# Roywangj/AdaptPoint

Measured on AMD Instinct MI355X. Metric: set-abstraction fwd+bwd point-clouds/sec (B=32,N=1024), higher is better.
Workload: dtype bf16

## Files before the change

### adaptpoint_amd/csrc/sa_fused.hip

```cpp
#include "apn_common.h"
#include "apn_mfma.h"
#include <type_traits>
#include "sa_chain.h"

namespace apn {

constexpr int SA_C = 32;
constexpr int SA_C1 = 32;
constexpr int SA_C2 = 64;
constexpr int SA_K = 32;
constexpr int SA_WAVES = 4;

template <int NS>
__device__ __forceinline__ void put_frag(uint4 *base, int f, int lane, const Frag<NS> &v) {
#pragma unroll
    for (int p = 0; p < NS; ++p) base[(f * NS + p) * 64 + lane] = __builtin_bit_cast(uint4, v.p[p]);
}

template <int NS>
__device__ __forceinline__ Frag<NS> get_frag(const uint4 *base, int f, int lane) {
    Frag<NS> v;
#pragma unroll
    for (int p = 0; p < NS; ++p) v.p[p] = __builtin_bit_cast(bf16x8, base[(f * NS + p) * 64 + lane]);
    return v;
}

template <int NS>
__device__ __forceinline__ float eff(float v) {
    const __bf16 hi = (__bf16)v;
    float r = (float)hi;
    if (NS == 2) r += (float)(__bf16)(v - r);
    return r;
}

struct SaArgs {
    int b, n, m;
    const float *xyz;
    const float *new_xyz;
    const __bf16 *ft;
    const __bf16 *ft_lo;
    const int *idx;
    const float *w1;
    float radius;
    const int *tmap;
    unsigned long long *stamps;
};

__device__ __forceinline__ void stamp(const SaArgs &a, int wave, int k) {
    if (a.stamps && (threadIdx.x & 63) == 0)
        a.stamps[((size_t)blockIdx.x * SA_WAVES + wave) * 16 + k] = wall_clock64();
}

__device__ __forceinline__ int tm_tiles(const SaArgs &a) { return a.tmap[0]; }
__device__ __forceinline__ const int *tm_tq0(const SaArgs &a) { return a.tmap + 4; }
__device__ __forceinline__ const unsigned *tm_rows(const SaArgs &a) {
    return reinterpret_cast<const unsigned *>(a.tmap + 4 + ((a.b * a.m + 3) & ~3));
}
__device__ __forceinline__ const int *tm_nn(const SaArgs &a) {
    return a.tmap + 4 + ((a.b * a.m + 3) & ~3) + (size_t)32 * a.b * a.m;
}
__device__ __forceinline__ unsigned ri_q(unsigned info) { return info & 0xffu; }
__device__ __forceinline__ unsigned ri_slot(unsigned info) { return (info >> 8) & 0xffu; }
__device__ __forceinline__ unsigned ri_mult(unsigned info) { return (info >> 16) & 0xffu; }
__device__ __forceinline__ void row_meta(unsigned info, int h, unsigned (&meta)[16]) {
#pragma unroll
    for (int i = 0; i < 16; ++i) meta[i] = (unsigned)__builtin_amdgcn_ds_bpermute(acc_row(i, h) << 2, (int)info);
}

template <int NS>
__device__ __forceinline__ void load_w1_frags(const float *__restrict__ w1, int r, int h,
                                              Frag<NS> (&wf)[3]) {
#pragma unroll
    for (int s = 0; s < 3; ++s) {
        float t[8];
#pragma unroll
        for (int j = 0; j < 8; ++j)
            t[j] = s < 2 ? w1[r * 35 + 3 + 16 * s + 8 * h + j]
                         : ((h == 0 && j < 3) ? w1[r * 35 + j] : 0.0f);
        wf[s] = make_frag<NS>(t);
    }
}

constexpr int PS_PTS = 512, PS_MAX_ROWS = 64, PS_NT = 2 * PS_PTS;
constexpr double GEO_INV_UNIT = 1.0 / 68719476736.0;

#ifdef APN_WG_STAMPS
__device__ unsigned long long *d_wg_stamps_f = nullptr;
__device__ __forceinline__ void wg_stamp(int k) {
    unsigned long long *st = d_wg_stamps_f;
    if (st && threadIdx.x == 0) st[(size_t)blockIdx.x * 16 + k] = wall_clock64();
}
#else
__device__ __forceinline__ void wg_stamp(int) {}
#endif

template <int NS>
__global__ __launch_bounds__(PS_NT) void sa_prep_stats_kernel(
    int n, int tiles_per_cloud, int total_tiles, const float *__restrict__ f, const long long *__restrict__ geo,
    const double *__restrict__ dd, int dd_rows, const float *__restrict__ w1, int stats, __bf16 *__restrict__ ft,
    __bf16 *__restrict__ ft_lo, float *__restrict__ part, unsigned long long *__restrict__ zero, long long zero_words) {
    extern __shared__ float sf_raw[];
    float (*sf)[PS_PTS + 1] = reinterpret_cast<float (*)[PS_PTS + 1]>(sf_raw);
    __shared__ float4 sgeo[PS_PTS];
    __shared__ float red[PS_NT / 64][64];
    __shared__ double sdd[6];
    const int tid = threadIdx.x, lane = tid & 63, r = lane & 31, h = lane >> 5;
    const int wave = __builtin_amdgcn_readfirstlane(tid >> 6);
    critical_stream_priority();
    wg_stamp(0);
    for (long long e = (long long)blockIdx.x * PS_NT + tid; e < zero_words; e += (long long)gridDim.x * PS_NT) zero[e] = 0ull;
    Frag<NS> wf[3];
    load_w1_frags<NS>(w1, r, h, wf);
    const float wp0 = eff<NS>(w1[r * 35]), wp1 = eff<NS>(w1[r * 35 + 1]), wp2 = eff<NS>(w1[r * 35 + 2]);
    float s1 = 0.0f, s2 = 0.0f;
    for (int tile = blockIdx.x; tile < total_tiles; tile += gridDim.x) {
        const int cloud = tile / tiles_per_cloud, n0 = (tile % tiles_per_cloud) * PS_PTS;
        {
            const int pt = tid & (PS_PTS - 1), cg = tid / PS_PTS;
            const bool in = n0 + pt < n;
            float v[16];
#pragma unroll
            for (int k = 0; k < 16; ++k) v[k] = in ? f[((size_t)cloud * SA_C + cg + 2 * k) * n + n0 + pt] : 0.0f;
            float4 gv = make_float4(0.f, 0.f, 0.f, 0.f);
            if (stats && in && cg == 0) {
                const longlong2 *gp = reinterpret_cast<const longlong2 *>(geo + ((size_t)cloud * n + n0 + pt) * 4);
                const longlong2 g0 = gp[0], g1 = gp[1];
                gv = make_float4((float)g0.x, (float)((double)g0.y * GEO_INV_UNIT), (float)((double)g1.x * GEO_INV_UNIT),
                                 (float)((double)g1.y * GEO_INV_UNIT));
            }
            wg_stamp(1);
            __syncthreads();
#pragma unroll
            for (int k = 0; k < 16; ++k) sf[cg + 2 * k][pt] = v[k];
            if (cg == 0) sgeo[pt] = gv;
            wg_stamp(2);
        }
        __syncthreads();
        wg_stamp(3);
        const int pt = 32 * wave + r;
        float x0[8], x1[8];
#pragma unroll
        for (int j = 0; j < 8; ++j) { x0[j] = sf[8 * h + j][pt]; x1[j] = sf[16 + 8 * h + j][pt]; }
        const Frag<NS> a0 = make_frag<NS>(x0), a1 = make_frag<NS>(x1);
        if (n0 + pt < n) {
            uint4 *row = reinterpret_cast<uint4 *>(ft + ((size_t)cloud * n + n0 + pt) * SA_C);
            row[h] = __builtin_bit_cast(uint4, a0.p[0]);
            row[2 + h] = __builtin_bit_cast(uint4, a1.p[0]);
            if (NS == 2) {
                uint4 *rl = reinterpret_cast<uint4 *>(ft_lo + ((size_t)cloud * n + n0 + pt) * SA_C);
                rl[h] = __builtin_bit_cast(uint4, a0.p[NS - 1]);
                rl[2 + h] = __builtin_bit_cast(uint4, a1.p[NS - 1]);
            }
        }
        wg_stamp(4);
        if (stats) {
            f32x16 y = {0};
            y = mfma<NS>(a0, wf[0], y);
            y = mfma<NS>(a1, wf[1], y);
#pragma unroll
            for (int i = 0; i < 16; ++i) {
                const float4 g = sgeo[32 * wave + acc_row(i, h)];
                const float PD = __builtin_fmaf(wp2, g.w, __builtin_fmaf(wp1, g.z, wp0 * g.y));
                const float oF = g.x * y[i];
                s1 += oF + PD;
                s2 += __builtin_fmaf(oF, y[i], 2.0f * y[i] * PD);
            }
        }
    }
    wg_stamp(5);
    if (!stats) return;
    s1 += __shfl_xor(s1, 32);
    s2 += __shfl_xor(s2, 32);
    if (lane < 32) { red[wave][r] = s1; red[wave][32 + r] = s2; }
    if (blockIdx.x == 0 && wave >= 1 && wave < 7) {
        double s = 0.0;
        for (int e = lane; e < dd_rows; e += 64) s += dd[(size_t)e * 6 + (wave - 1)];
#pragma unroll
        for (int o = 32; o > 0; o >>= 1) s += __shfl_xor(s, o);
        if (lane == 0) sdd[wave - 1] = s;
    }
    __syncthreads();
    if (tid < 64) {
        float val = 0.0f;
#pragma unroll
        for (int w = 0; w < PS_NT / 64; ++w) val += red[w][tid];
        if (tid >= 32 && blockIdx.x == 0) {
            const double wx = wp0, wy = wp1, wz = wp2;
            const double t = wx * wx * sdd[0] + 2.0 * wx * wy * sdd[1] + 2.0 * wx * wz * sdd[2] + wy * wy * sdd[3] +
                             2.0 * wy * wz * sdd[4] + wz * wz * sdd[5];
            val += (float)t;
        }
        part[(size_t)blockIdx.x * 64 + tid] = val;
    }
    wg_stamp(6);
}

template <int NS>
struct TileRaw {
    uint4 f[2], fl[NS];
    float px, py, pz;
    float qx, qy, qz;
    int nb;
    unsigned info;
    int q0;
};

struct TileHead {
    int nb, q0;
    unsigned info;
    int tile;
};
template <bool CP>
__device__ __forceinline__ TileHead load_head(const SaArgs &a, int tile, int r) {
    TileHead t;
    t.tile = tile;
    if (CP) {
        t.nb = tm_nn(a)[(size_t)tile * SA_K + r];
        t.info = tm_rows(a)[(size_t)tile * SA_K + r];
        t.q0 = tm_tq0(a)[tile];
    } else {
        t.nb = a.idx[(size_t)tile * SA_K + r];
        t.info = 0x10000u | ((unsigned)r << 8);
        t.q0 = tile;
    }
    return t;
}

template <typename T>
__device__ __forceinline__ T ld_off(const void *base, unsigned byte_off) {
    return *reinterpret_cast<const T *>(reinterpret_cast<const char *>(base) + byte_off);
}

template <int NS>
__device__ __forceinline__ void fetch_tile(const SaArgs &a, const TileHead &hd, int h, TileRaw<NS> &t) {
    const int nb = hd.nb;
    const unsigned cloud = (unsigned)(hd.q0 / a.m);
    const unsigned pt = cloud * (unsigned)a.n + (unsigned)nb;
    const unsigned rowoff = pt * (unsigned)(SA_C * 2) + 16u * (unsigned)h;
    t.f[0] = ld_off<uint4>(a.ft, rowoff);
    t.f[1] = ld_off<uint4>(a.ft, rowoff + 32u);
    if (NS == 2) {
        t.fl[0] = ld_off<uint4>(a.ft_lo, rowoff);
        t.fl[NS - 1] = ld_off<uint4>(a.ft_lo, rowoff + 32u);
    }
    struct xyz3 { float x, y, z; };
    const xyz3 pp = ld_off<xyz3>(a.xyz, pt * 12u);
    t.px = pp.x; t.py = pp.y; t.pz = pp.z;
    const unsigned q = (unsigned)hd.q0 + (ri_mult(hd.info) ? ri_q(hd.info) : 0u);
    const xyz3 qq = ld_off<xyz3>(a.new_xyz, q * 12u);
    t.qx = qq.x; t.qy = qq.y; t.qz = qq.z;
    t.nb = nb;
    t.info = hd.info;
    t.q0 = hd.q0;
}

template <int NS>
__device__ __forceinline__ void build_frags(const SaArgs &a, const TileRaw<NS> &t, int h,
                                            Frag<NS> (&x)[3], float *deff = nullptr) {
    x[0].p[0] = __builtin_bit_cast(bf16x8, t.f[0]);
    x[1].p[0] = __builtin_bit_cast(bf16x8, t.f[1]);
    if (NS == 2) {
        x[0].p[NS - 1] = __builtin_bit_cast(bf16x8, t.fl[0]);
        x[1].p[NS - 1] = __builtin_bit_cast(bf16x8, t.fl[NS - 1]);
    }
    float d[8] = {0.f, 0.f, 0.f, 0.f, 0.f, 0.f, 0.f, 0.f};
    if (h == 0 || deff) {
        d[0] = (t.px - t.qx) / a.radius;
        d[1] = (t.py - t.qy) / a.radius;
        d[2] = (t.pz - t.qz) / a.radius;
    }
    if (deff) {
#pragma unroll
        for (int j = 0; j < 3; ++j) {
            const __bf16 hi = (__bf16)d[j];
            deff[j] = (float)hi;
            if (NS == 2) deff[j] += (float)(__bf16)(d[j] - (float)hi);
        }
        if (h != 0) d[0] = d[1] = d[2] = 0.0f;
    }
    x[2] = make_frag<NS>(d);
}

__device__ __forceinline__ void touch(const TileHead &hd) {
    asm volatile("" ::"v"(hd.nb), "v"(hd.info), "v"(hd.q0));
}

struct NoAhead {
    __device__ __forceinline__ void operator()(const TileHead &) const {}
};
template <int NS, bool CP, bool LATE = false, typename Pro, typename Pre, typename Body, typename Ahead = NoAhead>
__device__ __forceinline__ void for_each_tile(const SaArgs &a, int wave, int r, int h, Pro prologue, Pre pre, Body body,
                                              Ahead ahead = Ahead()) {
    const int cap = a.b * a.m, stride = gridDim.x * SA_WAVES;
    const int tiles = CP ? tm_tiles(a) : cap;
    const bool xcd = (gridDim.x & 7) == 0;
    const int per_x = (tiles + 7) >> 3;
    auto remap = [&](int t) {
        if (!xcd) return t;
        const int wg = t / SA_WAVES, wv = t - wg * SA_WAVES;
        const int x = wg & 7, u = (wg >> 3) * SA_WAVES + wv;
        return u < per_x ? x * per_x + u : tiles;
    };
    int slot = blockIdx.x * SA_WAVES + wave;
    int tile = remap(slot);
    const TileHead hd0 = load_head<CP>(a, tile < tiles ? tile : 0, r);
    TileHead hd_nxt = load_head<CP>(a, remap(slot + stride) < tiles ? remap(slot + stride) : 0, r);
    TileRaw<NS> cur, nxt;
    const bool any = tile < tiles;
    stamp(a, wave, 1);
    if (any) {
        ahead(hd0);
        fetch_tile<NS>(a, hd0, h, cur);
    }
    prologue();
    stamp(a, wave, 2);
    if (!any) return;
    int nst = 3;
    for (; tile < tiles; slot += stride, tile = remap(slot)) {
        const bool more = remap(slot + stride) < tiles;
        const int tile2 = remap(slot + 2 * stride);
        if (LATE) {
            const TileHead hd_nxt2 = load_head<CP>(a, tile2 < tiles ? tile2 : tile, r);
            body(tile, cur, nst == 4, [&] {
                asm volatile("" ::: "memory");
                touch(hd_nxt);
                if (more) {
                    ahead(hd_nxt);
                    fetch_tile<NS>(a, hd_nxt, h, cur);
                }
            });
            stamp(a, wave, nst < 5 ? nst : 5);
            ++nst;
            hd_nxt = hd_nxt2;
            continue;
        }
        touch(hd_nxt);
        pre();
        if (more) fetch_tile<NS>(a, hd_nxt, h, nxt);
        const TileHead hd_nxt2 = load_head<CP>(a, tile2 < tiles ? tile2 : tile, r);
        body(tile, cur, nst == 4, [&] { touch(hd_nxt2); });
        stamp(a, wave, nst < 5 ? nst : 5);
        ++nst;
        if (more) cur = nxt;
        hd_nxt = hd_nxt2;
    }
    pre();
    stamp(a, wave, 6);
}

template <int NV>
__device__ __forceinline__ float fold_partials(float (&vals)[NV], int lane, int wave) {
    __shared__ float red[SA_WAVES][NV][32];
#pragma unroll
    for (int i = 0; i < NV; ++i) {
        const float other = __shfl_xor(vals[i], 32);
        if (lane < 32) red[wave][i][lane] = vals[i] + other;
    }
    __syncthreads();
    float s = 0.0f;
    const int e = threadIdx.x;
    if (e < NV * 32) {
#pragma unroll
        for (int w = 0; w < SA_WAVES; ++w) s += red[w][e >> 5][e & 31];
    }
    return s;
}

__device__ __forceinline__ void fold_rows32(const float *__restrict__ part, int rows, const double *__restrict__ sums,
                                            const BnArgs &bn, float *__restrict__ pack, float &scale, float &shift,
                                            double *scratch ) {
    double (*fred)[64] = reinterpret_cast<double (*)[64]>(scratch);
    double *ftot = scratch + 16 * 64;
    const int tid = threadIdx.x;
    double count = bn.count;
    double gpre = 1.0, bpre = 0.0;
    if (tid < 32) {
        if (bn.gamma) gpre = (double)bn.gamma[tid];
        if (bn.beta) bpre = (double)bn.beta[tid];
    }
    if (bn.training) {
        if (part) {
            const int quad = tid & 15, rg = tid >> 4;
            const float4 *__restrict__ p4 = reinterpret_cast<const float4 *>(part) + quad;
            double s0 = 0.0, s1 = 0.0, s2 = 0.0, s3 = 0.0;
            int rr = rg;
            for (; rr + 7 * 16 < rows; rr += 8 * 16) {
                float4 v[8];
#pragma unroll
                for (int u = 0; u < 8; ++u) v[u] = p4[(size_t)(rr + 16 * u) * 16];
#pragma unroll
                for (int u = 0; u < 8; ++u) {
                    s0 += (double)v[u].x; s1 += (double)v[u].y; s2 += (double)v[u].z; s3 += (double)v[u].w;
                }
            }
            for (; rr + 3 * 16 < rows; rr += 4 * 16) {
                float4 v[4];
#pragma unroll
                for (int u = 0; u < 4; ++u) v[u] = p4[(size_t)(rr + 16 * u) * 16];
#pragma unroll
                for (int u = 0; u < 4; ++u) {
                    s0 += (double)v[u].x; s1 += (double)v[u].y; s2 += (double)v[u].z; s3 += (double)v[u].w;
                }
            }
            for (; rr < rows; rr += 16) {
                const float4 v = p4[(size_t)rr * 16];
                s0 += (double)v.x; s1 += (double)v.y; s2 += (double)v.z; s3 += (double)v.w;
            }
            fred[rg][4 * quad] = s0; fred[rg][4 * quad + 1] = s1; fred[rg][4 * quad + 2] = s2; fred[rg][4 * quad + 3] = s3;
            __syncthreads();
            if (tid < 64) {
                double s = 0.0;
#pragma unroll
                for (int k = 0; k < 16; ++k) s += fred[k][tid];
                ftot[tid] = s;
            }
        } else if (tid < 64) {
            ftot[tid] = sums[tid];
        }
        if (!part) count = sums[64];
        __syncthreads();
    }
    if (tid < 32) {
        if (tid == 0 && blockIdx.x == 0 && bn.training && bn.nbt) *bn.nbt += 1;
        bn_channel(bn, 32, tid, bn.training ? ftot[tid] : 0.0, bn.training ? ftot[32 + tid] : 0.0, count,
                   blockIdx.x == 0, pack, scale, shift, gpre, bpre);
    }
}

template <int NS, bool CP>
__global__ __launch_bounds__(SA_WAVES * 64, 3) void sa_fwd_main_kernel(
    SaArgs a, const float *__restrict__ w2, BnArgs bn1, const float *__restrict__ part1, int rows1,
    const double *__restrict__ sums1, float *__restrict__ pack1, const float *__restrict__ gamma2,
    float *__restrict__ ysel, unsigned char *__restrict__ ksel, unsigned long long *__restrict__ acc2) {
    const int lane = threadIdx.x & 63, r = lane & 31, h = lane >> 5;
    const int wave = __builtin_amdgcn_readfirstlane(threadIdx.x >> 6);
    enum { F_W1 = 0, F_W2 = 3, F_COUNT = 7 };
    __shared__ uint4 cfrag[F_COUNT * NS * 64];
    __shared__ __attribute__((aligned(16))) float bn1v[2][2][16];
    constexpr int PT_WAVE = CP ? 2 * 32 * 33 : 17 * 64 * 2 / SA_WAVES;
    __shared__ __attribute__((aligned(16))) float ptile[SA_WAVES * PT_WAVE];
    __shared__ __attribute__((aligned(16))) unsigned sinfo[SA_WAVES][32];
    static_assert(SA_WAVES * PT_WAVE * 4 >= 17 * 64 * 8, "fold scratch");
    critical_stream_priority();
    stamp(a, wave, 0);
    const float sg[2] = {(!gamma2 || gamma2[r] >= 0.0f) ? 1.0f : -1.0f, (!gamma2 || gamma2[32 + r] >= 0.0f) ? 1.0f : -1.0f};
    float st[4] = {0.0f, 0.0f, 0.0f, 0.0f};

    auto prologue = [&]() {
        if (wave == 0) {
            Frag<NS> w1f[3];
            load_w1_frags<NS>(a.w1, r, h, w1f);
#pragma unroll
            for (int s = 0; s < 3; ++s) put_frag<NS>(cfrag, F_W1 + s, lane, w1f[s]);
        }
        if (wave == 1 || wave == 2) {
            const int t = wave - 1;
#pragma unroll
            for (int s = 0; s < 2; ++s) {
                float tmp[8];
#pragma unroll
                for (int j = 0; j < 8; ++j) tmp[j] = w2[(32 * t + r) * SA_C1 + acc_row(8 * s + j, h)];
                put_frag<NS>(cfrag, F_W2 + 2 * t + s, lane, make_frag<NS>(tmp));
            }
        }
        float sc, sh;
        fold_rows32(part1, rows1, sums1, bn1, pack1, sc, sh, reinterpret_cast<double *>(ptile));
        if (threadIdx.x < 32) {
            const int i = threadIdx.x;
            bn1v[0][(i >> 2) & 1][(i & 3) + 4 * (i >> 3)] = sc;
            bn1v[1][(i >> 2) & 1][(i & 3) + 4 * (i >> 3)] = sh;
        }
        __syncthreads();
    };

    for_each_tile<NS, CP>(a, wave, r, h, prologue, [] {}, [&](int tile, const TileRaw<NS> &raw, bool, auto before_stores) {
        int lane_o = lane;
        asm volatile("" : "+v"(lane_o));
        Frag<NS> x[3];
        build_frags<NS>(a, raw, h, x);
        const int q0 = __builtin_amdgcn_readfirstlane(raw.q0);
        const int nq = __builtin_amdgcn_readfirstlane((int)(raw.info >> 24));
        float multf[16];
        unsigned starts = 1u;
        float *pt = ptile + wave * PT_WAVE;
        if (CP) {
            if (lane < 32) sinfo[wave][lane] = raw.info;
#pragma unroll
            for (int gq = 0; gq < 4; ++gq) {
                const uint4 v = *reinterpret_cast<const uint4 *>(&sinfo[wave][8 * gq + 4 * (lane_o >> 5)]);
                multf[4 * gq] = (float)ri_mult(v.x); multf[4 * gq + 1] = (float)ri_mult(v.y);
                multf[4 * gq + 2] = (float)ri_mult(v.z); multf[4 * gq + 3] = (float)ri_mult(v.w);
            }
            const unsigned prev = (unsigned)__shfl_up((int)raw.info, 1);
            starts = (unsigned)__ballot(lane < 32 && (lane == 0 || ri_q(raw.info) != ri_q(prev)));
        }
        f32x16 y1 = {0};
#pragma unroll
        for (int s = 0; s < 3; ++s) y1 = mfma<NS>(get_frag<NS>(cfrag, F_W1 + s, lane_o), x[s], y1);
        {
            const float4 *scv = reinterpret_cast<const float4 *>(bn1v[0][lane_o >> 5]);
            const float4 *shv = reinterpret_cast<const float4 *>(bn1v[1][lane_o >> 5]);
#pragma unroll
            for (int i4 = 0; i4 < 4; ++i4) {
                const float4 sc = scv[i4], sh = shv[i4];
                y1[4 * i4] = __builtin_fmaxf(__builtin_fmaf(y1[4 * i4], sc.x, sh.x), 0.0f);
                y1[4 * i4 + 1] = __builtin_fmaxf(__builtin_fmaf(y1[4 * i4 + 1], sc.y, sh.y), 0.0f);
                y1[4 * i4 + 2] = __builtin_fmaxf(__builtin_fmaf(y1[4 * i4 + 2], sc.z, sh.z), 0.0f);
                y1[4 * i4 + 3] = __builtin_fmaxf(__builtin_fmaf(y1[4 * i4 + 3], sc.w, sh.w), 0.0f);
            }
        }
        const Frag<NS> a0 = pack8<NS>(y1, 0), a1 = pack8<NS>(y1, 8);
#pragma unroll
        for (int t = 0; t < 2; ++t) {
            f32x16 y2 = {0};
            y2 = mfma<NS>(a0, get_frag<NS>(cfrag, F_W2 + 2 * t, lane_o), y2);
            y2 = mfma<NS>(a1, get_frag<NS>(cfrag, F_W2 + 2 * t + 1, lane_o), y2);
            if (CP) {
                float s1 = 0.0f, s2 = 0.0f;
#pragma unroll
                for (int i = 0; i < 16; ++i) {
                    const float wy = multf[i] * y2[i];
                    s1 += wy;
                    s2 += wy * y2[i];
                    pt[(t * 32 + acc_row(i, h)) * 33 + r] = sg[t] * y2[i];
                }
                st[t] += s1;
                st[2 + t] += s2;
                continue;
            }
            float best = sg[t] * y2[0];
            int bpos = 0;
            float s1 = 0.0f, s2 = 0.0f;
#pragma unroll
            for (int i = 0; i < 16; ++i) {
                s1 += y2[i];
                s2 += y2[i] * y2[i];
                const float v = sg[t] * y2[i];
                if (i > 0 && v > best) { best = v; bpos = i; }
            }
            st[t] += s1;
            st[2 + t] += s2;
            int kpos = acc_row(bpos, h);
            const float obest = __shfl_xor(best, 32);
            const int okpos = __shfl_xor(kpos, 32);
            if (obest > best || (obest == best && okpos < kpos)) { best = obest; kpos = okpos; }
            if (h == 0) {
                ysel[(size_t)tile * SA_C2 + 32 * t + r] = sg[t] * best;
                ksel[(size_t)tile * SA_C2 + 32 * t + r] = (unsigned char)kpos;
            }
        }
        if (CP) {
            asm volatile("" ::: "memory");
            const float *mine = pt + h * (32 * 33) + r;
            const float sgn = h ? sg[1] : sg[0];
            float *ys = ysel + (size_t)q0 * SA_C2 + lane;
            unsigned char *ks = ksel + (size_t)q0 * SA_C2 + lane;
            before_stores();
            int seg = -1, ra = 0, kpos = 0;
            float best = 0.0f;
#pragma unroll
            for (int half16 = 0; half16 < 2; ++half16) {
                float v[16];
#pragma unroll
                for (int i = 0; i < 16; ++i) v[i] = mine[(16 * half16 + i) * 33];
#pragma unroll
                for (int i = 0; i < 16; ++i) {
                    const int rho = 16 * half16 + i;
                    if ((starts >> rho) & 1u) {
                        if (seg >= 0 && seg < nq) {
                            ys[(size_t)seg * SA_C2] = sgn * best;
                            ks[(size_t)seg * SA_C2] = (unsigned char)kpos;
                        }
                        ++seg;
                        best = -__builtin_inff();
                        kpos = 0;
                        ra = rho;
                    }
                    const bool up = v[i] > best;
                    best = up ? v[i] : best;
                    kpos = up ? rho - ra : kpos;
                }
            }
            if (seg >= 0 && seg < nq) {
                ys[(size_t)seg * SA_C2] = sgn * best;
                ks[(size_t)seg * SA_C2] = (unsigned char)kpos;
            }
            asm volatile("" ::: "memory");
        }
    });
    const float tot = fold_partials<4>(st, lane, wave);
    if (threadIdx.x < 128) acc_add(acc2, 128, blockIdx.x % ACC_COPIES, threadIdx.x, tot);
    stamp(a, wave, 7);
}

struct SaBwdArgs {
    const float *w2;
    const float *scale1, *shift1, *mean1, *inv1;
    const float *pack2;
    const unsigned long long *accS;
    const double *sumsS;
    double count;
    int train2;
    const float *goa;
    const unsigned char *ksel;
    const int *rowdst;
};

template <int NS, bool CP>
__global__ __launch_bounds__(SA_WAVES * 64, 2) void sa_bwd_kernel(SaArgs a, SaBwdArgs g,
                                                               unsigned long long *__restrict__ accT,
                                                               float *__restrict__ partW2,
                                                               float *__restrict__ GU,
                                                               float *__restrict__ HA,
                                                               float *__restrict__ HB) {
    static_assert(CP, "the backward pass runs over a tile map");
    const int lane = threadIdx.x & 63, r = lane & 31, h = lane >> 5;
    const int wave = __builtin_amdgcn_readfirstlane(threadIdx.x >> 6);
    enum { F_W1 = 0, F_QM = 3, F_W2T = 5, F_COUNT = 9 };
    __shared__ uint4 cfrag[F_COUNT * NS * 64];
    __shared__ __attribute__((aligned(16))) float bn1v[2][2][16];
    __shared__ __attribute__((aligned(16))) float sw2[SA_C2][SA_C1 + 4];
    __shared__ float sD[SA_C2], sE[SA_C2];
    __shared__ __attribute__((aligned(16))) float sqm[SA_C1 + 1][SA_C1 + 4];
    critical_stream_priority();
    stamp(a, wave, 0);
    __shared__ float chan[5][32];
    f32x16 dsp[2] = {{0}, {0}};
    f32x16 gram = {0};
    float suma = 0.0f;
    float st[2] = {0.0f, 0.0f};

    constexpr int SP_ROW = 72, SP_TILE = 32 * SP_ROW;
    constexpr int SP_WAVE = (CP && NS * SP_TILE * 2 < 2 * 32 * 33 * 4) ? 2 * 32 * 33 * 4 : NS * SP_TILE * 2;
    constexpr int SP_BYTES = SA_WAVES * SP_WAVE, WRED_BYTES = SA_WAVES * SA_C2 * SA_C1 * 4;
    __shared__ __attribute__((aligned(16))) unsigned char sp_raw[SP_BYTES > WRED_BYTES ? SP_BYTES : WRED_BYTES];
    __shared__ __attribute__((aligned(16))) unsigned sinfo[SA_WAVES][32];
    __shared__ __attribute__((aligned(16))) float qgoa[CP ? SA_WAVES : 1][4 * SA_C2];
    __shared__ __attribute__((aligned(16))) unsigned char qksel[CP ? SA_WAVES : 1][4 * SA_C2];
    __bf16 *sp_img = reinterpret_cast<__bf16 *>(sp_raw + wave * SP_WAVE);

    __shared__ __attribute__((aligned(16))) int sdst[SA_WAVES][2][64];
    int ahead_n = 0, body_n = 0;
    auto gu_store = [&](int place, float v) {
        *reinterpret_cast<float *>(reinterpret_cast<char *>(GU) + (((unsigned)place << 7) + ((unsigned)r << 2))) = v;
    };

    auto prologue = [&]() {
        const int tid = threadIdx.x;
        {
            Frag<NS> w1f[3];
            if (wave == 0) load_w1_frags<NS>(a.w1, r, h, w1f);
            float wv[8];
#pragma unroll
            for (int k = 0; k < 8; ++k) wv[k] = g.w2[tid + 256 * k];
            float c1[4] = {0.f, 0.f, 0.f, 0.f};
            if (tid >= 128 && tid < 160) {
                c1[0] = g.scale1[tid - 128]; c1[1] = g.shift1[tid - 128]; c1[2] = g.mean1[tid - 128]; c1[3] = g.inv1[tid - 128];
            }
            double sv = 0.0, count = g.count;
            float p_sc = 0.0f, p_mu = 0.0f, p_iv = 0.0f;
            if (tid < 128) sv = g.sumsS ? g.sumsS[tid] : acc_read(g.accS, 128, tid);
            if (g.sumsS) count = g.sumsS[128];
            if (tid < 64) { p_sc = g.pack2[tid]; p_mu = g.pack2[128 + tid]; p_iv = g.pack2[192 + tid]; }
            if (wave == 0) {
#pragma unroll
                for (int s = 0; s < 3; ++s) put_frag<NS>(cfrag, F_W1 + s, lane, w1f[s]);
            }
#pragma unroll
            for (int k = 0; k < 8; ++k) sw2[(tid + 256 * k) >> 5][tid & 31] = wv[k];
            if (tid >= 128 && tid < 160) {
#pragma unroll
                for (int k = 0; k < 4; ++k) chan[k][tid - 128] = c1[k];
            }
            double *sS2 = reinterpret_cast<double *>(&sqm[0][0]);
            if (tid >= 64 && tid < 128) sS2[tid - 64] = sv;
            __syncthreads();
            if (tid < 64) {
                const double sc = p_sc, mu = p_mu, iv = p_iv, s1 = sv, s2 = sS2[tid];
                double d = 0.0, e = 0.0;
                if (g.train2) {
                    const double rc = 1.0 / count;
                    d = -sc * iv * s2 * rc;
                    e = (-sc * s1 + sc * mu * iv * s2) * rc;
                }
                sD[tid] = (float)d;
                sE[tid] = (float)e;
            }
            if (tid >= 64 && tid < 96) {
                const int i = tid - 64;
                const float sci = g.scale1[i], shi = g.shift1[i];
                bn1v[0][(i >> 2) & 1][(i & 3) + 4 * (i >> 3)] = sci;
                bn1v[1][(i >> 2) & 1][(i & 3) + 4 * (i >> 3)] = shi;
            }
        }
        __syncthreads();
        {
            const int s = wave;
            float tmp[8], tmpd[8], tmpe[8];
#pragma unroll
            for (int j = 0; j < 8; ++j) {
                const int c = 16 * s + 8 * h + j;
                tmp[j] = sw2[c][r];
                tmpd[j] = tmp[j] * sD[c];
                tmpe[j] = r == 0 ? sE[c] : 0.0f;
            }
            const Frag<NS> wt = make_frag<NS>(tmp);
            put_frag<NS>(cfrag, F_W2T + s, lane, wt);
            const f32x16 zero16 = {0};
            const f32x16 qp = mfma<NS>(make_frag<NS>(tmpd), wt, zero16);
            const f32x16 ep = mfma<NS>(make_frag<NS>(tmpe), wt, zero16);
            float *scr = reinterpret_cast<float *>(sp_img);
#pragma unroll
            for (int e = 0; e < 16; ++e) scr[e * 64 + lane] = qp[e];
            if (h == 0) scr[16 * 64 + r] = ep[0];
        }
        __syncthreads();
        if (wave == 2) {
            f32x16 qacc = {0};
            float ev = 0.0f;
#pragma unroll
            for (int w = 0; w < SA_WAVES; ++w) {
                const float *pw = reinterpret_cast<const float *>(sp_raw + w * SP_WAVE);
#pragma unroll
                for (int e = 0; e < 16; ++e) qacc[e] += pw[e * 64 + lane];
                if (h == 0) ev += pw[16 * 64 + r];
            }
            put_frag<NS>(cfrag, F_QM, lane, pack8<NS>(qacc, 0));
            put_frag<NS>(cfrag, F_QM + 1, lane, pack8<NS>(qacc, 8));
            if (h == 0) chan[4][r] = ev;
        }
        __syncthreads();
        {
            uint4 *z = reinterpret_cast<uint4 *>(sp_img);
            for (int e = lane; e < SP_WAVE / 16; e += 64) z[e] = make_uint4(0u, 0u, 0u, 0u);
        }
    };

    auto scatter_pending = [] {};
    auto ahead = [&](const TileHead &hd) {
        if (!CP) return;
        typedef __attribute__((address_space(3))) void lds_void;
        typedef __attribute__((address_space(1))) const void glb_void;
        const int q0n = __builtin_amdgcn_readfirstlane(hd.q0);
        const int qbn = q0n < a.b * a.m - 4 ? q0n : a.b * a.m - 4;
        int l_o = lane;
        asm volatile("" : "+v"(l_o));
        const char *gb = reinterpret_cast<const char *>(g.goa) + (size_t)qbn * (SA_C2 * 4);
        const char *kb = reinterpret_cast<const char *>(g.ksel) + (size_t)qbn * SA_C2;
        __builtin_amdgcn_global_load_lds((glb_void *)(gb + (unsigned)(16 * l_o)), (lds_void *)&qgoa[wave][0], 16, 0, 0);
        __builtin_amdgcn_global_load_lds((glb_void *)(kb + (unsigned)(4 * l_o)), (lds_void *)&qksel[wave][0], 4, 0, 0);
        const char *db = reinterpret_cast<const char *>(g.rowdst) + (size_t)__builtin_amdgcn_readfirstlane(hd.tile) * (SA_K * 4);
        __builtin_amdgcn_global_load_lds((glb_void *)(db + (unsigned)(4 * (l_o & 31))), (lds_void *)&sdst[wave][ahead_n & 1][0], 4, 0, 0);
        ++ahead_n;
    };
    for_each_tile<NS, CP, CP>(a, wave, r, h, prologue, scatter_pending, [&](int tile, const TileRaw<NS> &raw, bool probe, auto before_stores) {
        auto st2 = [&](int k) { if (probe) stamp(a, wave, 8 + k); };
        st2(0);
        int lane_o = lane;
        asm volatile("" : "+v"(lane_o));
        Frag<NS> x[3];
        build_frags<NS>(a, raw, h, x);

        const int q0 = __builtin_amdgcn_readfirstlane(raw.q0);
        const int nq = CP ? __builtin_amdgcn_readfirstlane((int)(raw.info >> 24)) : 1;
        const bool live_row = !CP || ri_mult(raw.info) != 0;
        const float mrow = CP ? (float)ri_mult(raw.info) : 1.0f;
        float gv4[4];
        int kc4[4];
        const int qb = q0 < a.b * a.m - 4 ? q0 : a.b * a.m - 4;
#pragma unroll
        for (int u = 0; u < 4; ++u) {
            if (CP) {
                gv4[u] = 0.0f;
                kc4[u] = 0;
            } else {
                gv4[u] = 0.0f;
                kc4[u] = 0;
                if (u == 0) {
                    gv4[u] = g.goa[(size_t)(q0 + u) * SA_C2 + lane];
                    kc4[u] = g.ksel[(size_t)(q0 + u) * SA_C2 + lane];
                }
            }
        }
        unsigned mpk[4] = {0x01010101u, 0x01010101u, 0x01010101u, 0x01010101u};
        unsigned starts = 1u;
        if (CP) {
            if (lane < 32) sinfo[wave][lane] = raw.info;
#pragma unroll
            for (int gq = 0; gq < 4; ++gq) {
                const uint4 v = *reinterpret_cast<const uint4 *>(&sinfo[wave][8 * gq + 4 * (lane_o >> 5)]);
                mpk[gq] = ri_mult(v.x) | (ri_mult(v.y) << 8) | (ri_mult(v.z) << 16) | (ri_mult(v.w) << 24);
            }
            const unsigned prev = (unsigned)__shfl_up((int)raw.info, 1);
            starts = (unsigned)__ballot(lane < 32 && (lane == 0 || ri_q(raw.info) != ri_q(prev)));
        }
        auto multf = [&](int i) { return (float)((mpk[i >> 2] >> (8 * (i & 3))) & 0xffu); };
        f32x16 yT = {0}, y1 = {0};
#pragma unroll
        for (int s = 0; s < 3; ++s) {
            const Frag<NS> w = get_frag<NS>(cfrag, F_W1 + s, lane_o);
            yT = mfma<NS>(w, x[s], yT);
            y1 = mfma<NS>(x[s], w, y1);
        }
        {
            const float4 *scv = reinterpret_cast<const float4 *>(bn1v[0][lane_o >> 5]);
            const float4 *shv = reinterpret_cast<const float4 *>(bn1v[1][lane_o >> 5]);
#pragma unroll
            for (int i4 = 0; i4 < 4; ++i4) {
                const float4 sc = scv[i4], sh = shv[i4];
                yT[4 * i4] = __builtin_fmaxf(__builtin_fmaf(yT[4 * i4], sc.x, sh.x), 0.0f);
                yT[4 * i4 + 1] = __builtin_fmaxf(__builtin_fmaf(yT[4 * i4 + 1], sc.y, sh.y), 0.0f);
                yT[4 * i4 + 2] = __builtin_fmaxf(__builtin_fmaf(yT[4 * i4 + 2], sc.z, sh.z), 0.0f);
                yT[4 * i4 + 3] = __builtin_fmaxf(__builtin_fmaf(yT[4 * i4 + 3], sc.w, sh.w), 0.0f);
            }
        }
        st2(1);
        Frag<NS> a0, a1;
        if (CP) {
            f32x16 yw;
#pragma unroll
            for (int i = 0; i < 16; ++i) yw[i] = yT[i] * mrow;
            a0 = pack8<NS>(yw, 0);
            a1 = pack8<NS>(yw, 8);
        } else {
            a0 = pack8<NS>(yT, 0);
            a1 = pack8<NS>(yT, 8);
        }

        Frag<NS> sp[4];
        {
            unsigned todo = starts;
            if (CP) {
                asm volatile("s_waitcnt vmcnt(0)" ::: "memory");
                const int dq = q0 - qb;
#pragma unroll
                for (int u = 0; u < 4; ++u) {
                    const int e = (u + dq < 4 ? u + dq : 3) * SA_C2 + lane_o;
                    gv4[u] = qgoa[wave][e];
                    kc4[u] = qksel[wave][e];
                }
            }
#pragma unroll 1
            for (int jb = 0; jb < nq; jb += 4) {
                if (jb) {
#pragma unroll
                    for (int u = 0; u < 4; ++u)
                        if (jb + u < nq) {
                            gv4[u] = g.goa[(size_t)(q0 + jb + u) * SA_C2 + lane];
                            kc4[u] = g.ksel[(size_t)(q0 + jb + u) * SA_C2 + lane];
                        }
                }
#pragma unroll
                for (int u = 0; u < 4; ++u) {
                    if (jb + u < nq) {
                        const float gv = gv4[u];
                        int kc = kc4[u];
                        if (CP) {
                            kc += __builtin_ctz(todo);
                            todo &= todo - 1u;
                        }
                        const __bf16 ghi = (__bf16)gv;
                        const __bf16 glo = (__bf16)(gv - (float)ghi);
                        __bf16 *cell = sp_img + kc * SP_ROW + lane;
                        cell[0] = ghi;
                        if (NS == 2) cell[SP_TILE] = glo;
                        if (!CP) kc4[u] = kc;
                    }
                }
            }
        }
        asm volatile("" ::: "memory");
        {
            f32x16 an;
            const float sc1 = chan[0][lane_o & 31], sh1 = chan[1][lane_o & 31];
#pragma unroll
            for (int i = 0; i < 16; ++i) {
                an[i] = __builtin_fmaxf(__builtin_fmaf(y1[i], sc1, sh1), 0.0f);
                if (CP) suma = __builtin_fmaf(multf(i), an[i], suma);
                else suma += an[i];
            }
            const Frag<NS> b0 = pack8<NS>(an, 0), b1 = pack8<NS>(an, 8);
            if (CP) {
                f32x16 aw;
#pragma unroll
                for (int i = 0; i < 16; ++i) aw[i] = an[i] * multf(i);
                gram = mfma<NS>(pack8<NS>(aw, 0), b0, gram);
                gram = mfma<NS>(pack8<NS>(aw, 8), b1, gram);
            } else {
                gram = mfma<NS>(b0, b0, gram);
                gram = mfma<NS>(b1, b1, gram);
            }
            typedef short tr_s4 __attribute__((ext_vector_type(4)));
            typedef short tr_s8 __attribute__((ext_vector_type(8)));
            typedef __attribute__((address_space(3))) tr_s4 tr_lds;
            const int li = lane_o & 15, gq = li >> 2, gp = li & 3, grh = (lane_o >> 4) & 1;
            const __bf16 *tb = sp_img + (4 * (lane_o >> 5) + gq) * SP_ROW + 16 * grh + 4 * gp;
#pragma unroll
            for (int t = 0; t < 2; ++t) {
#pragma unroll
                for (int sk = 0; sk < 2; ++sk) {
                    Frag<NS> at;
#pragma unroll
                    for (int pp = 0; pp < NS; ++pp) {
                        const __bf16 *src = tb + pp * SP_TILE + (16 * sk) * SP_ROW + 32 * t;
                        const tr_s4 lo4 = __builtin_amdgcn_ds_read_tr16_b64_v4i16((tr_lds *)(src));
                        const tr_s4 hi4 = __builtin_amdgcn_ds_read_tr16_b64_v4i16((tr_lds *)(src + 8 * SP_ROW));
                        const tr_s8 v8 = {lo4.x, lo4.y, lo4.z, lo4.w, hi4.x, hi4.y, hi4.z, hi4.w};
                        at.p[pp] = __builtin_bit_cast(bf16x8, v8);
                    }
                    dsp[t] = mfma<NS>(at, sk ? b1 : b0, dsp[t]);
                }
            }
        }
        st2(2);
#pragma unroll
        for (int s = 0; s < 4; ++s) {
            const __bf16 *src = sp_img + r * SP_ROW + 16 * s + 8 * h;
            sp[s].p[0] = *reinterpret_cast<const bf16x8 *>(src);
            if (NS == 2) sp[s].p[NS - 1] = *reinterpret_cast<const bf16x8 *>(src + SP_TILE);
        }
        asm volatile("" ::: "memory");
        if (!CP) {
            __bf16 *cell = sp_img + kc4[0] * SP_ROW + lane;
            cell[0] = (__bf16)0.0f;
            if (NS == 2) cell[SP_TILE] = (__bf16)0.0f;
        }
        f32x16 ga;
        const float ev = chan[4][lane_o & 31];
#pragma unroll
        for (int i = 0; i < 16; ++i) ga[i] = CP ? ev * multf(i) : ev;
        ga = mfma<NS>(a0, get_frag<NS>(cfrag, F_QM, lane_o), ga);
        ga = mfma<NS>(a1, get_frag<NS>(cfrag, F_QM + 1, lane_o), ga);
#pragma unroll
        for (int s = 0; s < 4; ++s) ga = mfma<NS>(sp[s], get_frag<NS>(cfrag, F_W2T + s, lane_o), ga);

        st2(3);
        float *gt = reinterpret_cast<float *>(sp_img);
        asm volatile("" ::: "memory");
        float s1 = 0.0f, s2 = 0.0f, hb = 0.0f;
        const float sc1l = chan[0][lane_o & 31], sh1l = chan[1][lane_o & 31], iv1 = chan[3][lane_o & 31];
        const float nmi = -chan[2][lane_o & 31] * iv1;
#pragma unroll
        for (int i = 0; i < 16; ++i) {
            const float u = __builtin_fmaf(y1[i], sc1l, sh1l);
            const float yhat = __builtin_fmaf(y1[i], iv1, nmi);
            ga[i] = u > 0.0f ? ga[i] : 0.0f;
            s1 += ga[i];
            s2 += ga[i] * yhat;
            if (CP) {
                gt[acc_row(i, h) * 33 + r] = ga[i];
                gt[32 * 33 + acc_row(i, h) * 33 + r] = multf(i) * yhat;
            } else {
                hb += yhat;
            }
        }
        st[0] += s1;
        st[1] += s2;

        st2(4);
        before_stores();
        {
            int live;
            if (CP) {
                asm volatile("" ::: "memory");
                const float *mine = gt + h * (32 * 33) + r;
                float *dst = (h ? HB : HA) + (size_t)q0 * SA_C1 + r;
                int seg = -1;
                float sum = 0.0f;
#pragma unroll
                for (int half16 = 0; half16 < 2; ++half16) {
                    float v[16];
#pragma unroll
                    for (int i = 0; i < 16; ++i) v[i] = mine[(16 * half16 + i) * 33];
#pragma unroll
                    for (int i = 0; i < 16; ++i) {
                        if ((starts >> (16 * half16 + i)) & 1u) {
                            if (seg >= 0 && seg < nq) dst[(size_t)seg * SA_C1] = sum;
                            ++seg;
                            sum = 0.0f;
                        }
                        sum += v[i];
                    }
                }
                if (seg >= 0 && seg < nq) dst[(size_t)seg * SA_C1] = sum;
                asm volatile("" ::: "memory");
                {
                    uint4 *z = reinterpret_cast<uint4 *>(sp_img);
#pragma unroll
                    for (int e = 0; e < (NS * SP_TILE * 2 / 16 + 63) / 64; ++e)
                        if (e * 64 + lane < NS * SP_TILE * 2 / 16) z[e * 64 + lane] = make_uint4(0u, 0u, 0u, 0u);
                }
                asm volatile("" ::: "memory");
                live = __popcll(__ballot(lane < 32 && live_row));
            } else {
                const float ha = s1 + __shfl_xor(s1, 32);
                hb += __shfl_xor(hb, 32);
                if (h == 0) {
                    HA[(size_t)tile * SA_C1 + r] = ha;
                    HB[(size_t)tile * SA_C1 + r] = hb;
                }
                live = 0;
            }

            st2(5);
            st2(6);
            if (CP) {
                const int *dl = &sdst[wave][body_n & 1][0];
#pragma unroll
                for (int gq = 0; gq < 4; ++gq) {
                    if (8 * gq < live) {
                        const int4 dd = *reinterpret_cast<const int4 *>(&dl[8 * gq + 4 * (lane_o >> 5)]);
                        const int base = 8 * gq + 4 * h;
                        if (base + 0 < live) gu_store(dd.x, ga[4 * gq + 0]);
                        if (base + 1 < live) gu_store(dd.y, ga[4 * gq + 1]);
                        if (base + 2 < live) gu_store(dd.z, ga[4 * gq + 2]);
                        if (base + 3 < live) gu_store(dd.w, ga[4 * gq + 3]);
                    }
                }
            }
            ++body_n;
        }
    }, ahead);
    {
        const float tot = fold_partials<2>(st, lane, wave);
        if (threadIdx.x < 64) acc_add(accT, 64, blockIdx.x % ACC_COPIES, threadIdx.x, tot);
    }
    float (*wred)[SA_C2 * SA_C1] = reinterpret_cast<float (*)[SA_C2 * SA_C1]>(sp_raw);
    __syncthreads();
#pragma unroll
    for (int i = 0; i < 16; ++i) {
        wred[wave][acc_row(i, h) * SA_C1 + r] = dsp[0][i];
        wred[wave][(32 + acc_row(i, h)) * SA_C1 + r] = dsp[1][i];
    }
    __syncthreads();
    const int ec = threadIdx.x >> 2, emid = (threadIdx.x & 3) * 8;
    float sp8[8];
    {
        float4 lo4 = make_float4(0.f, 0.f, 0.f, 0.f), hi4 = lo4;
#pragma unroll
        for (int w = 0; w < SA_WAVES; ++w) {
            const float4 a4 = *reinterpret_cast<const float4 *>(&wred[w][ec * SA_C1 + emid]);
            const float4 b4 = *reinterpret_cast<const float4 *>(&wred[w][ec * SA_C1 + emid + 4]);
            lo4.x += a4.x; lo4.y += a4.y; lo4.z += a4.z; lo4.w += a4.w;
            hi4.x += b4.x; hi4.y += b4.y; hi4.z += b4.z; hi4.w += b4.w;
        }
        sp8[0] = lo4.x; sp8[1] = lo4.y; sp8[2] = lo4.z; sp8[3] = lo4.w;
        sp8[4] = hi4.x; sp8[5] = hi4.y; sp8[6] = hi4.z; sp8[7] = hi4.w;
    }
    __syncthreads();
    suma += __shfl_xor(suma, 32);
#pragma unroll
    for (int i = 0; i < 16; ++i) wred[wave][acc_row(i, h) * SA_C1 + r] = gram[i];
    if (h == 0) wred[wave][SA_C1 * SA_C1 + r] = suma;
    __syncthreads();
    for (int e = threadIdx.x; e < SA_C1 * SA_C1 + SA_C1; e += SA_WAVES * 64)
        sqm[e >> 5][e & 31] = (wred[0][e] + wred[1][e]) + (wred[2][e] + wred[3][e]);
    __syncthreads();
    {
        float acc[8];
#pragma unroll
        for (int j = 0; j < 8; ++j) acc[j] = 0.0f;
#pragma unroll 8
        for (int k = 0; k < SA_C1; ++k) {
            const float w = sw2[ec][k];
            const float4 g0 = *reinterpret_cast<const float4 *>(&sqm[k][emid]);
            const float4 g1 = *reinterpret_cast<const float4 *>(&sqm[k][emid + 4]);
            acc[0] = __builtin_fmaf(w, g0.x, acc[0]); acc[1] = __builtin_fmaf(w, g0.y, acc[1]);
            acc[2] = __builtin_fmaf(w, g0.z, acc[2]); acc[3] = __builtin_fmaf(w, g0.w, acc[3]);
            acc[4] = __builtin_fmaf(w, g1.x, acc[4]); acc[5] = __builtin_fmaf(w, g1.y, acc[5]);
            acc[6] = __builtin_fmaf(w, g1.z, acc[6]); acc[7] = __builtin_fmaf(w, g1.w, acc[7]);
        }
        const float d = sD[ec], e = sE[ec];
        const float4 s0 = *reinterpret_cast<const float4 *>(&sqm[32][emid]);
        const float4 s1 = *reinterpret_cast<const float4 *>(&sqm[32][emid + 4]);
        float4 *row = reinterpret_cast<float4 *>(partW2 + (size_t)blockIdx.x * (SA_C2 * SA_C1) + ec * SA_C1 + emid);
        row[0] = make_float4(sp8[0] + d * acc[0] + e * s0.x, sp8[1] + d * acc[1] + e * s0.y,
                             sp8[2] + d * acc[2] + e * s0.z, sp8[3] + d * acc[3] + e * s0.w);
        row[1] = make_float4(sp8[4] + d * acc[4] + e * s1.x, sp8[5] + d * acc[5] + e * s1.y,
                             sp8[6] + d * acc[6] + e * s1.z, sp8[7] + d * acc[7] + e * s1.w);
    }
    stamp(a, wave, 7);
}

static int sa_grid(int tiles, bool compact = false) {
    const int cap = compact ? 768 : 512;
    int g = (tiles + SA_WAVES - 1) / SA_WAVES;
    return g < cap ? (g < 1 ? 1 : g) : cap;
}

static int sa_grid_bwd(int tiles) {
    int g = sa_grid(tiles);
    return g < 448 ? g : 448;
}

}

extern "C" int apn_sa_grid_blocks(int b, int m) { return apn::sa_grid(b * m); }
extern "C" int apn_sa_grid_rows(int b, int m, int with_tile_map) { return apn::sa_grid(b * m, with_tile_map != 0); }
extern "C" int apn_sa_bwd_main_rows(int b, int m) { return apn::sa_grid_bwd(b * m); }
extern "C" int apn_sa_acc_words(int ncol) { return ncol > 0 ? apn::acc_words(ncol) : 0; }

extern "C" int apn_sa_prep_rows(int b, int n) {
    const long long tiles = (long long)b * ((n + apn::PS_PTS - 1) / apn::PS_PTS);
    return (int)(tiles < apn::PS_MAX_ROWS ? (tiles < 1 ? 1 : tiles) : apn::PS_MAX_ROWS);
}

extern "C" int apn_sa_prep_stats(int b, int n, const float *f, const void *geo, const void *dd, const float *w1,
                                 int precision, int stats, void *ft, float *part1, void *zero, long long zero_words,
                                 void *stream) {
    using namespace apn;
    if (b <= 0 || n <= 0 || b > 65535 || (precision != 1 && precision != 2) || !f || !ft || !w1) return APN_EINVAL;
    if (stats && (!geo || !dd || !part1 || ((uintptr_t)geo & 15) || ((uintptr_t)part1 & 15))) return APN_EINVAL;
    if (zero_words < 0 || (zero_words && !zero)) return APN_EINVAL;
    __bf16 *hi = (__bf16 *)ft;
    __bf16 *lo = precision == 2 ? hi + (size_t)b * n * SA_C : nullptr;
    const int tpc = (n + PS_PTS - 1) / PS_PTS;
    auto kern = precision == 2 ? sa_prep_stats_kernel<2> : sa_prep_stats_kernel<1>;
    const int lds = SA_C * (PS_PTS + 1) * (int)sizeof(float);
    static DynLdsOnce lds_set[2];
    if (hipError_t e = set_dyn_lds(lds_set[precision - 1], (const void *)kern, lds)) return (int)e;
    hipLaunchKernelGGL(kern, dim3(apn_sa_prep_rows(b, n)), dim3(PS_NT), lds, (hipStream_t)stream, n, tpc, b * tpc, f,
                       (const long long *)geo, (const double *)dd, b * (apn_sa_geo_dd_doubles(n) / 6), w1, stats, hi, lo, part1,
                       (unsigned long long *)zero, zero_words);
    APN_LAUNCH_CHECK();
    return APN_OK;
}

#ifdef APN_WG_STAMPS
extern "C" __attribute__((visibility("default"))) int apn_sa_debug_wg_stamps_fused(void *buf) {
    return (int)hipMemcpyToSymbol(HIP_SYMBOL(apn::d_wg_stamps_f), &buf, sizeof(buf));
}
#endif

static unsigned long long *g_stamps = nullptr;
extern "C" int apn_sa_debug_stamps(void *buf) { g_stamps = (unsigned long long *)buf; return APN_OK; }

static apn::SaArgs sa_args(int b, int n, int m, const float *xyz, const float *new_xyz, const void *ft,
                           int precision, const int *idx, const float *w1, float radius, const int *tmap) {
    const __bf16 *hi = (const __bf16 *)ft;
    return apn::SaArgs{b, n, m, xyz, new_xyz, hi,
                       precision == 2 ? hi + (size_t)b * n * apn::SA_C : nullptr, idx, w1, radius, tmap, g_stamps};
}

static int sa_check(int b, int n, int m, int precision) {
    if (precision != 1 && precision != 2) return APN_EINVAL;
    if (b <= 0 || n <= 0 || m <= 0) return APN_EINVAL;
    if ((long long)b * m > 0x7fffffffLL / 64) return APN_EINVAL;
    if ((long long)b * n > 0xffffffffLL / 256) return APN_EINVAL;
    if ((long long)b * m > 0xffffffffLL / (32 * 128)) return APN_EINVAL;
    return APN_OK;
}

extern "C" int apn_sa_fwd_main(int b, int n, int m, int precision, float radius, const float *xyz,
                               const float *new_xyz, const void *ft, const int *idx, const int *tmap, const float *w1,
                               const float *w2, const float *g1, const float *b1, float *rm1, float *rv1, void *nbt1,
                               float eps1, float mom1, int train1, double count, const float *part1, int rows1,
                               const double *sums1, float *pack1, const float *gamma2, float *ysel, void *ksel,
                               void *acc2, void *stream) {
    using namespace apn;
    if (int e = sa_check(b, n, m, precision)) return e;
    if (!xyz || !new_xyz || !ft || !idx || !w1 || !w2 || !pack1 || !ysel || !ksel || !acc2) return APN_EINVAL;
    if (train1 && !part1 && !sums1) return APN_EINVAL;
    if (!train1 && (!rm1 || !rv1)) return APN_EINVAL;
    if (part1 && (((uintptr_t)part1 & 15) || rows1 <= 0)) return APN_EINVAL;
    SaArgs a = sa_args(b, n, m, xyz, new_xyz, ft, precision, idx, w1, radius, tmap);
    BnArgs bn{g1, b1, rm1, rv1, (long long *)nbt1, eps1, mom1, train1, count};
    auto kern = precision == 2 ? (tmap ? sa_fwd_main_kernel<2, true> : sa_fwd_main_kernel<2, false>)
                               : (tmap ? sa_fwd_main_kernel<1, true> : sa_fwd_main_kernel<1, false>);
    hipLaunchKernelGGL(kern, dim3(sa_grid(b * m, tmap != nullptr)), dim3(SA_WAVES * 64), 0, (hipStream_t)stream, a, w2, bn,
                       sums1 ? nullptr : part1, rows1, sums1, pack1, gamma2, ysel, (unsigned char *)ksel,
                       (unsigned long long *)acc2);
    APN_LAUNCH_CHECK();
    return APN_OK;
}

extern "C" int apn_sa_bwd_main(int b, int n, int m, int precision, float radius, const float *xyz,
                               const float *new_xyz, const void *ft, const int *idx, const int *tmap, const float *w1,
                               const float *w2, const float *pack1, const float *pack2, const void *accS,
                               const double *sumsS, double count, int train2, const float *goa, const void *ksel,
                               void *accT, float *partW2, const int *rowdst, float *GU, float *HA, float *HB, void *stream) {
    using namespace apn;
    if (int e = sa_check(b, n, m, precision)) return e;
    if (!w2 || !pack1 || !pack2 || (!accS && !sumsS) || !goa || !ksel || !accT || !partW2 || !GU || !HA || !HB)
        return APN_EINVAL;
    if (!tmap || !rowdst) return APN_EINVAL;
    SaArgs a = sa_args(b, n, m, xyz, new_xyz, ft, precision, idx, w1, radius, tmap);
    SaBwdArgs g;
    g.w2 = w2;
    g.scale1 = pack1; g.shift1 = pack1 + 32; g.mean1 = pack1 + 64; g.inv1 = pack1 + 96;
    g.pack2 = pack2;
    g.accS = (const unsigned long long *)accS; g.sumsS = sumsS;
    g.count = count; g.train2 = train2;
    g.goa = goa; g.ksel = (const unsigned char *)ksel;
    g.rowdst = rowdst;
    auto kern = precision == 2 ? sa_bwd_kernel<2, true> : sa_bwd_kernel<1, true>;
    hipLaunchKernelGGL(kern, dim3(sa_grid_bwd(b * m)), dim3(SA_WAVES * 64), 0, (hipStream_t)stream, a, g,
                       (unsigned long long *)accT, partW2, GU, HA, HB);
    APN_LAUNCH_CHECK();
    return APN_OK;
}
```

Measured before the change: 122,300.

## Derive transposed activation fragments via LDS transpose instead of recomputing MFMAs

Removes the second set of three layer-1 MFMAs (yT) and the separate BN/ReLU pass that produced the transposed activation fragments in the backward kernel. The already-weighted activations (aw0/aw1) are written to the per-wave LDS image in a swizzled layout and read back with ds_read_tr16 transpose loads to form a0/a1. This reuses the computed activations and drops the bn1v shared table, at the cost of extra LDS stores and loads plus a reuse of the scratch region that may add latency or hazards.

```diff
diff --git a/adaptpoint_amd/csrc/sa_fused.hip b/adaptpoint_amd/csrc/sa_fused.hip
--- a/adaptpoint_amd/csrc/sa_fused.hip
+++ b/adaptpoint_amd/csrc/sa_fused.hip
@@ -618,7 +618,6 @@
     const int wave = __builtin_amdgcn_readfirstlane(threadIdx.x >> 6);
     enum { F_W1 = 0, F_QM = 3, F_W2T = 5, F_COUNT = 9 };
     __shared__ uint4 cfrag[F_COUNT * NS * 64];
-    __shared__ __attribute__((aligned(16))) float bn1v[2][2][16];
     __shared__ __attribute__((aligned(16))) float sw2[SA_C2][SA_C1 + 4];
     __shared__ float sD[SA_C2], sE[SA_C2];
     __shared__ __attribute__((aligned(16))) float sqm[SA_C1 + 1][SA_C1 + 4];
@@ -685,12 +684,6 @@
                 }
                 sD[tid] = (float)d;
                 sE[tid] = (float)e;
-            }
-            if (tid >= 64 && tid < 96) {
-                const int i = tid - 64;
-                const float sci = g.scale1[i], shi = g.shift1[i];
-                bn1v[0][(i >> 2) & 1][(i & 3) + 4 * (i >> 3)] = sci;
-                bn1v[1][(i >> 2) & 1][(i & 3) + 4 * (i >> 3)] = shi;
             }
         }
         __syncthreads();
@@ -764,7 +757,6 @@
         const int q0 = __builtin_amdgcn_readfirstlane(raw.q0);
         const int nq = CP ? __builtin_amdgcn_readfirstlane((int)(raw.info >> 24)) : 1;
         const bool live_row = !CP || ri_mult(raw.info) != 0;
-        const float mrow = CP ? (float)ri_mult(raw.info) : 1.0f;
         float gv4[4];
         int kc4[4];
         const int qb = q0 < a.b * a.m - 4 ? q0 : a.b * a.m - 4;
@@ -795,37 +787,10 @@
             starts = (unsigned)__ballot(lane < 32 && (lane == 0 || ri_q(raw.info) != ri_q(prev)));
         }
         auto multf = [&](int i) { return (float)((mpk[i >> 2] >> (8 * (i & 3))) & 0xffu); };
-        f32x16 yT = {0}, y1 = {0};
-#pragma unroll
-        for (int s = 0; s < 3; ++s) {
-            const Frag<NS> w = get_frag<NS>(cfrag, F_W1 + s, lane_o);
-            yT = mfma<NS>(w, x[s], yT);
-            y1 = mfma<NS>(x[s], w, y1);
-        }
-        {
-            const float4 *scv = reinterpret_cast<const float4 *>(bn1v[0][lane_o >> 5]);
-            const float4 *shv = reinterpret_cast<const float4 *>(bn1v[1][lane_o >> 5]);
-#pragma unroll
-            for (int i4 = 0; i4 < 4; ++i4) {
-                const float4 sc = scv[i4], sh = shv[i4];
-                yT[4 * i4] = __builtin_fmaxf(__builtin_fmaf(yT[4 * i4], sc.x, sh.x), 0.0f);
-                yT[4 * i4 + 1] = __builtin_fmaxf(__builtin_fmaf(yT[4 * i4 + 1], sc.y, sh.y), 0.0f);
-                yT[4 * i4 + 2] = __builtin_fmaxf(__builtin_fmaf(yT[4 * i4 + 2], sc.z, sh.z), 0.0f);
-                yT[4 * i4 + 3] = __builtin_fmaxf(__builtin_fmaf(yT[4 * i4 + 3], sc.w, sh.w), 0.0f);
-            }
-        }
+        f32x16 y1 = {0};
+#pragma unroll
+        for (int s = 0; s < 3; ++s) y1 = mfma<NS>(x[s], get_frag<NS>(cfrag, F_W1 + s, lane_o), y1);
         st2(1);
-        Frag<NS> a0, a1;
-        if (CP) {
-            f32x16 yw;
-#pragma unroll
-            for (int i = 0; i < 16; ++i) yw[i] = yT[i] * mrow;
-            a0 = pack8<NS>(yw, 0);
-            a1 = pack8<NS>(yw, 8);
-        } else {
-            a0 = pack8<NS>(yT, 0);
-            a1 = pack8<NS>(yT, 8);
-        }
 
         Frag<NS> sp[4];
         {
@@ -870,6 +835,7 @@
             }
         }
         asm volatile("" ::: "memory");
+        Frag<NS> aw0, aw1;
         {
             f32x16 an;
             const float sc1 = chan[0][lane_o & 31], sh1 = chan[1][lane_o & 31];
@@ -884,12 +850,14 @@
                 f32x16 aw;
 #pragma unroll
                 for (int i = 0; i < 16; ++i) aw[i] = an[i] * multf(i);
-                gram = mfma<NS>(pack8<NS>(aw, 0), b0, gram);
-                gram = mfma<NS>(pack8<NS>(aw, 8), b1, gram);
+                aw0 = pack8<NS>(aw, 0);
+                aw1 = pack8<NS>(aw, 8);
             } else {
-                gram = mfma<NS>(b0, b0, gram);
-                gram = mfma<NS>(b1, b1, gram);
-            }
+                aw0 = b0;
+                aw1 = b1;
+            }
+            gram = mfma<NS>(aw0, b0, gram);
+            gram = mfma<NS>(aw1, b1, gram);
             typedef short tr_s4 __attribute__((ext_vector_type(4)));
             typedef short tr_s8 __attribute__((ext_vector_type(8)));
             typedef __attribute__((address_space(3))) tr_s4 tr_lds;
@@ -924,6 +892,43 @@
             __bf16 *cell = sp_img + kc4[0] * SP_ROW + lane;
             cell[0] = (__bf16)0.0f;
             if (NS == 2) cell[SP_TILE] = (__bf16)0.0f;
+        }
+        Frag<NS> a0, a1;
+        {
+            typedef short tr_s4 __attribute__((ext_vector_type(4)));
+            typedef short tr_s8 __attribute__((ext_vector_type(8)));
+            typedef __attribute__((address_space(3))) tr_s4 tr_lds;
+            constexpr int TP_PLANE = 32 * 64;
+            static_assert(NS * TP_PLANE <= SP_WAVE && NS * TP_PLANE <= NS * SP_TILE * 2, "the planes fit the image's region");
+            char *pl = reinterpret_cast<char *>(sp_img);
+            const int lr = lane_o & 31, lh = lane_o >> 5;
+            const int wo = 64 * lr + 8 * (lh ^ ((lr >> 1) & 7));
+#pragma unroll
+            for (int pp = 0; pp < NS; ++pp) {
+                const tr_s8 v0 = __builtin_bit_cast(tr_s8, aw0.p[pp]), v1 = __builtin_bit_cast(tr_s8, aw1.p[pp]);
+                *reinterpret_cast<tr_s4 *>(pl + pp * TP_PLANE + wo) = __builtin_shufflevector(v0, v0, 0, 1, 2, 3);
+                *reinterpret_cast<tr_s4 *>(pl + pp * TP_PLANE + (wo ^ 16)) = __builtin_shufflevector(v0, v0, 4, 5, 6, 7);
+                *reinterpret_cast<tr_s4 *>(pl + pp * TP_PLANE + (wo ^ 32)) = __builtin_shufflevector(v1, v1, 0, 1, 2, 3);
+                *reinterpret_cast<tr_s4 *>(pl + pp * TP_PLANE + (wo ^ 48)) = __builtin_shufflevector(v1, v1, 4, 5, 6, 7);
+            }
+            asm volatile("" ::: "memory");
+            const int li = lane_o & 15, gq = li >> 2, gp = li & 3, grh = (lane_o >> 4) & 1;
+            const int ro = 256 * lh + 64 * gq + 8 * ((4 * grh + gp) ^ (2 * lh + (gq >> 1)));
+            const char *t0 = pl + ro, *t1 = pl + (ro ^ 32) + 512;
+#pragma unroll
+            for (int sk = 0; sk < 2; ++sk) {
+                Frag<NS> at;
+#pragma unroll
+                for (int pp = 0; pp < NS; ++pp) {
+                    const tr_s4 lo4 = __builtin_amdgcn_ds_read_tr16_b64_v4i16((tr_lds *)(t0 + pp * TP_PLANE + 1024 * sk));
+                    const tr_s4 hi4 = __builtin_amdgcn_ds_read_tr16_b64_v4i16((tr_lds *)(t1 + pp * TP_PLANE + 1024 * sk));
+                    const tr_s8 v8 = {lo4.x, lo4.y, lo4.z, lo4.w, hi4.x, hi4.y, hi4.z, hi4.w};
+                    at.p[pp] = __builtin_bit_cast(bf16x8, v8);
+                }
+                if (sk) a1 = at;
+                else a0 = at;
+            }
+            asm volatile("" ::: "memory");
         }
         f32x16 ga;
         const float ev = chan[4][lane_o & 31];
```

Result: no change. 122,700, median of 6 (+0.3%).
